# winddori2002/DEX-TTS

Hardware: AMD Instinct MI355X
Metric: mel-frames/s at n_timesteps=50, 80-ch mel (sampler only); RTF (higher is better)
Workload: dtype bf16; 1 GPU; gedex_b1: gedex_lj B=1/GPU T=512 n_timesteps=50 (BASELINE.json configs[1]); global_batch=1, frames=512, hipgraph=False, parallelism=1 GPU

## Files before the change

dex_tts_amd/csrc/conv3x3_bf16.hip:

```cpp
#include "kernels.h"
#include <cstdlib>
#include <cstdio>
#include "lp_util.h"
#include "kernels_lp.h"
#include "conv_gn.h"

namespace dex {
namespace DEX_LP_NS {

typedef float f32x16 __attribute__((ext_vector_type(16)));
typedef unsigned short u16;
typedef unsigned u32x4 __attribute__((ext_vector_type(4)));

__device__ __forceinline__ float cv_mish(float x) {
    const float e = __expf(fminf(x, 20.f));
    const float n = e * (e + 2.f);
    return x * (n * __builtin_amdgcn_rcpf(n + 2.f));
}

template <int NT, int COUT>
__device__ __forceinline__ void cv_epilogue(const Conv3P& p, f32x16 (&acc)[NT], int b, int ho, int w0, int nbase, int lane, int tid,
                                            long long* gnred) {
    const int i = lane & 31, hh = lane >> 5;
    constexpr int cpg = COUT / 8;
    if (p.gn_stats) { if (tid < 16) gnred[tid] = 0; __syncthreads(); }
    const bool full = ho < p.H && w0 + 32 <= p.W;
    const long ybase = (long)b * p.H * p.W * COUT + ((long)ho * p.W + w0 + 4 * hh) * COUT + nbase + i;
    float* yl = p.Y + ybase;
    u16* yh = reinterpret_cast<u16*>(p.Y) + ybase;
    const bool yb = p.y_bf16 != 0;
#pragma unroll
    for (int t = 0; t < NT; ++t) {
        const int n = nbase + t * 32 + i;
        const float bias = p.bias[n];
        float gs = 0.f, gss = 0.f;
        if (full && yb) {
            const bool odd = (lane & 1) != 0;
            u16* yp = yh + (odd ? 16 * COUT - 1 : 0) + t * 32;
#pragma unroll
            for (int r = 0; r < 16; ++r) { const float v = acc[t][r] + bias; gs += v; gss = fmaf(v, v, gss); }
#pragma unroll
            for (int j = 0; j < 8; ++j) {
                const float lo_r = acc[t][j] + bias, hi_r = acc[t][8 + j] + bias;
                const float recv = lane_xor1(odd ? lo_r : hi_r);
                const float mine = odd ? hi_r : lo_r;
                const unsigned pk = odd ? pack2_lp(recv, mine) : pack2_lp(mine, recv);
                *reinterpret_cast<unsigned*>(yp + ((j & 3) + 8 * (j >> 2)) * COUT) = pk;
            }
        } else if (full) {
            const bool odd = (lane & 1) != 0;
            float* yp = yl + (odd ? 16 * COUT - 1 : 0) + t * 32;
#pragma unroll
            for (int r = 0; r < 16; ++r) { const float v = acc[t][r] + bias; gs += v; gss = fmaf(v, v, gss); }
#pragma unroll
            for (int j = 0; j < 8; ++j) {
                const float lo_r = acc[t][j] + bias, hi_r = acc[t][8 + j] + bias;
                const float recv = lane_xor1(odd ? lo_r : hi_r);
                const float mine = odd ? hi_r : lo_r;
                *reinterpret_cast<float2*>(yp + ((j & 3) + 8 * (j >> 2)) * COUT) = odd ? make_float2(recv, mine) : make_float2(mine, recv);
            }
        } else {
#pragma unroll
            for (int r = 0; r < 16; ++r) {
                const int wo = w0 + (r & 3) + 8 * (r >> 2) + 4 * hh;
                const bool ok = ho < p.H && wo < p.W;
                const float v = acc[t][r] + bias;
                const float vs = ok ? v : 0.f;
                gs += vs; gss = fmaf(vs, vs, gss);
                if (ok) {
                    if (yb) yh[((r & 3) + 8 * (r >> 2)) * COUT + t * 32] = lp_bits(v);
                    else yl[((r & 3) + 8 * (r >> 2)) * COUT + t * 32] = v;
                }
            }
        }
        if (p.gn_stats) {
            for (int o = 1; o < cpg; o <<= 1) { gs += __shfl_xor(gs, o); gss += __shfl_xor(gss, o); }
            gs += __shfl_xor(gs, 32); gss += __shfl_xor(gss, 32);
            if (hh == 0 && (i & (cpg - 1)) == 0) {
                const double inv_n = 1.0 / ((double)p.H * p.W * cpg);
                gn_add(&gnred[(n / cpg) * 2], gn_fix(gs, inv_n)); gn_add(&gnred[(n / cpg) * 2 + 1], gn_fix(gss, inv_n));
            }
        }
    }
    if (p.gn_stats) {
        __syncthreads();
        if (tid < 16) {
            const long long v = gnred[tid];
            if (v != 0) {
                const int slot = (blockIdx.x + blockIdx.y * gridDim.x) % GN_SLOTS;
                gn_add(p.gn_stats + (((long)b * 8 + (tid >> 1)) * GN_SLOTS + slot) * 2 + (tid & 1), v);
            }
        }
    }
}

template <int NT, int COUT>
__device__ __forceinline__ void cv_res_store(const Conv3P& p, const f32x16 (&accr)[NT], int b, int ho, int w0, int nb, int lane) {
    const int i = lane & 31, hh = lane >> 5;
    float* yl = p.res_y + ((long)b * p.H * p.W + (long)ho * p.W + w0 + 4 * hh) * COUT + nb + i;
    const bool rfull = ho < p.H && w0 + 32 <= p.W;
    const bool odd = (lane & 1) != 0;
#pragma unroll
    for (int t = 0; t < NT; ++t) {
        const float bias = p.res_b[nb + t * 32 + i];
        if (rfull) {
            float* yp = yl + (odd ? 16 * COUT - 1 : 0) + t * 32;
#pragma unroll
            for (int j = 0; j < 8; ++j) {
                const float lo_r = accr[t][j] + bias, hi_r = accr[t][8 + j] + bias;
                const float recv = lane_xor1(odd ? lo_r : hi_r);
                const float mine = odd ? hi_r : lo_r;
                *reinterpret_cast<float2*>(yp + ((j & 3) + 8 * (j >> 2)) * COUT) = odd ? make_float2(recv, mine) : make_float2(mine, recv);
            }
        } else {
#pragma unroll
            for (int r = 0; r < 16; ++r) {
                const int wo = w0 + (r & 3) + 8 * (r >> 2) + 4 * hh;
                if (ho < p.H && wo < p.W) yl[((r & 3) + 8 * (r >> 2)) * COUT + t * 32] = accr[t][r] + bias;
            }
        }
    }
}

template <int CC, int COUT, int NSL, int TH, bool PRO2 = false, bool RES = false, bool XB = false, int NW = 4>
__global__ __launch_bounds__(64 * NW) void conv3x3_lp_kernel(const Conv3P p) {
    constexpr int PW = 34, PH = TH + 2;
    constexpr int LDP = CC + 8;
    constexpr int WN = NW / TH;
    constexpr int NTHR = 64 * NW;
    constexpr int NT = NSL / 32 / WN;
    constexpr int NSLICE = COUT / NSL;
    constexpr int ITEMS = PH * PW * (CC / 8);
    constexpr int NI = (ITEMS + NTHR - 1) / NTHR;
    constexpr int WPT = NSL * CC / 8 / NTHR;
    constexpr int RING = CC == 128 ? (PRO2 ? 1 : 2) : 3;
    constexpr int NPASS = CC == 128 ? (TH == 8 ? (PRO2 ? 8 : 4) : (PRO2 ? 5 : 2)) : (PRO2 ? 3 : 1);
    constexpr int NIP = (NI + NPASS - 1) / NPASS;
#ifdef DEX_LP_WSPLIT
    constexpr int NTAP = 18;
#else
    constexpr int NTAP = 9;
#endif
    static_assert(NT >= 1 && WPT >= 1, "tile");
    extern __shared__ __attribute__((aligned(16))) u16 smem[];
    u16* patch = smem;
    u16* wbuf = smem + PH * PW * LDP;
    u16* rbuf = wbuf + 2 * NSL * LDP;
    __shared__ long long gnred[16];
    constexpr int COEF_N = (TH == 8) ? 128 : 256;
    __shared__ __attribute__((aligned(16))) float coef[3][COEF_N];

    const int tid = threadIdx.x, lane = tid & 63, wave = tid >> 6;
    const int i = lane & 31, hh = lane >> 5;
    const int wrow = wave % TH, wcol = wave / TH;
#ifdef DEX_TIMING
    long long tk[8] = {0, 0, 0, 0, 0, 0, 0, 0};
    const long long tk0 = __builtin_readcyclecounter();
    long long tlast = tk0;
#define CSTAMP(k) do { const long long now_ = __builtin_readcyclecounter(); tk[k] += now_ - tlast; tlast = now_; } while (0)
#else
#define CSTAMP(k) do {} while (0)
#endif
    const int xs = p.skip_dead ? (int)((blockIdx.x + blockIdx.y + blockIdx.z) % gridDim.x) : (int)blockIdx.x;
    const int w0 = xs * 32, h0 = blockIdx.y * TH;
    const int b = blockIdx.z / NSLICE, slice = blockIdx.z % NSLICE;
    const int step = p.step;
    const float* X = p.X + (long)b * p.H * p.W * p.ldx + p.x_coff;
    const u16* Xh = reinterpret_cast<const u16*>(p.X) + (long)b * p.H * p.W * p.ldx + p.x_coff;
    const float* mrow = p.mask + (long)b * p.mask_bstride;
    const int K = 9 * p.Cin;
    const u16* Wg = reinterpret_cast<const u16*>(p.Wbf) + (long)slice * NSL * K;
    const bool pro = p.pro_stats != nullptr;
    if constexpr (!PRO2) {
        if (p.skip_dead) {
            const int wi = w0 - 1 + (lane < 34 ? lane : 33);
            const float mv = (unsigned)wi < (unsigned)p.W ? mrow[wi * p.mask_ws] : 0.f;
            if (__builtin_amdgcn_ballot_w64(mv != 0.f) == 0) {
                f32x16 zacc[NT];
#pragma unroll
                for (int t = 0; t < NT; ++t)
#pragma unroll
                    for (int r = 0; r < 16; ++r) zacc[t][r] = 0.f;
                if constexpr (RES) cv_res_store<NT, COUT>(p, zacc, b, h0 + wrow, w0, slice * NSL + wcol * NT * 32, lane);
                cv_epilogue<NT, COUT>(p, zacc, b, h0 + wrow, w0, slice * NSL + wcol * NT * 32, lane, tid, gnred);
                return;
            }
        }
    }

    f32x16 acc[NT];
#pragma unroll
    for (int t = 0; t < NT; ++t)
#pragma unroll
        for (int r = 0; r < 16; ++r) acc[t][r] = 0.f;

    f32x16 accr[RES ? NT : 1];
    if constexpr (RES) {
#pragma unroll
        for (int t = 0; t < NT; ++t)
#pragma unroll
            for (int r = 0; r < 16; ++r) accr[t][r] = 0.f;
    }
    int wofs[WPT], wlds[WPT];
#pragma unroll
    for (int j = 0; j < WPT; ++j) {
        const int it = tid + NTHR * j;
        const int n = it / (CC / 8), c8 = (it % (CC / 8)) * 8;
        wofs[j] = n * K + c8;
        wlds[j] = n * LDP + c8;
    }
    const int pc8 = (tid % (CC / 8)) * 8;

    CvGnLoads gnl{};
    if (pro) gnl = cv_gn_issue(p, b, tid, step);
    const int nchunk = p.Cin / CC;
    for (int ch = 0; ch < nchunk; ++ch) {
        const int cbase = ch * CC;
        u32x4 w0r[WPT], wr[RING][WPT], rwr[RES ? WPT : 1];
#ifdef DEX_LP_WSPLIT
        u32x4 rwl[RES ? WPT : 1];
#define WS_TAPOFS(t) ((long)((t) % 9) * p.Cin + ((t) >= 9 ? p.w_lo_off : 0L))
#else
#define WS_TAPOFS(t) ((long)(t) * p.Cin)
#endif
        float4 sc0, sc1, sh0, sh1, t0, t1;
#pragma unroll
        for (int ps = 0; ps < NPASS; ++ps) {
            float4 pf0[NIP], pf1[XB ? 1 : NIP], rf0[PRO2 ? NIP : 1], rf1[PRO2 ? NIP : 1];
            float pmk[NIP];
            bool pin[NIP];
#pragma unroll
            for (int q = 0; q < NIP; ++q) {
                const int it = min(tid + NTHR * (ps * NIP + q), ITEMS - 1);
                const int px = it / (CC / 8);
                const int pw = px % PW, ph = px / PW;
                const int hi = h0 + ph - 1, wi = w0 + pw - 1;
                const bool inb = (unsigned)hi < (unsigned)p.H && (unsigned)wi < (unsigned)p.W;
                const int hc = inb ? hi : 0, wc = inb ? wi : 0;
                if constexpr (XB) {
                    pf0[q] = *reinterpret_cast<const float4*>(Xh + ((long)hc * p.W + wc) * p.ldx + cbase + pc8);
                } else {
                    const float* src = X + ((long)hc * p.W + wc) * p.ldx + cbase + pc8;
                    pf0[q] = *reinterpret_cast<const float4*>(src);
                    pf1[q] = *reinterpret_cast<const float4*>(src + 4);
                }
                if constexpr (PRO2) {
                    const float* rs = p.pro_res + ((long)b * p.H * p.W + (long)hc * p.W + wc) * p.Cin + cbase + pc8;
                    rf0[q] = *reinterpret_cast<const float4*>(rs);
                    rf1[q] = *reinterpret_cast<const float4*>(rs + 4);
                }
                const float mk = mrow[wc * p.mask_ws];
                pmk[q] = inb ? mk : 0.f;
                pin[q] = inb;
            }
            if (ps == 0) {
                if constexpr (RES) {
                    const u16* Rg = reinterpret_cast<const u16*>(p.res_w) + (long)slice * NSL * p.Cin;
#pragma unroll
                    for (int j = 0; j < WPT; ++j) {
                        const int it = tid + NTHR * j;
                        rwr[j] = *reinterpret_cast<const u32x4*>(Rg + (long)(it / (CC / 8)) * p.Cin + cbase + (it % (CC / 8)) * 8);
#ifdef DEX_LP_WSPLIT
                        rwl[j] = *reinterpret_cast<const u32x4*>(Rg + p.res_lo_off + (long)(it / (CC / 8)) * p.Cin + cbase + (it % (CC / 8)) * 8);
#endif
                    }
                }
#pragma unroll
                for (int j = 0; j < WPT; ++j) w0r[j] = *reinterpret_cast<const u32x4*>(Wg + wofs[j] + cbase);
#pragma unroll
                for (int s = 0; s < RING; ++s)
#pragma unroll
                    for (int j = 0; j < WPT; ++j) wr[s][j] = *reinterpret_cast<const u32x4*>(Wg + wofs[j] + WS_TAPOFS(s + 1) + cbase);
                CSTAMP(0);
                if (pro && ch == 0) cv_gn_finish<COEF_N>(p, gnl, tid, coef);
                __builtin_amdgcn_sched_barrier(0);
                lds_barrier();
                CSTAMP(1);
                if (pro) {
                    const int c = cbase + pc8;
                    sc0 = *reinterpret_cast<const float4*>(&coef[0][c]); sc1 = *reinterpret_cast<const float4*>(&coef[0][c + 4]);
                    sh0 = *reinterpret_cast<const float4*>(&coef[1][c]); sh1 = *reinterpret_cast<const float4*>(&coef[1][c + 4]);
                    t0 = *reinterpret_cast<const float4*>(&coef[2][c]); t1 = *reinterpret_cast<const float4*>(&coef[2][c + 4]);
                }
            }
#pragma unroll
            for (int q = 0; q < NIP; ++q) {
                float4 f0, f1;
                if constexpr (XB) {
                    const float4 r = pf0[q];
                    const unsigned u0 = __float_as_uint(r.x), u1 = __float_as_uint(r.y), u2 = __float_as_uint(r.z), u3 = __float_as_uint(r.w);
                    f0 = make_float4(lp_lo(u0), lp_hi(u0), lp_lo(u1), lp_hi(u1));
                    f1 = make_float4(lp_lo(u2), lp_hi(u2), lp_lo(u3), lp_hi(u3));
                } else { f0 = pf0[q]; f1 = pf1[q]; }
#ifdef DEX_SCALAR_PROLOGUE
                if (pro) {
                    f0.x = cv_mish(fmaf(f0.x, sc0.x, sh0.x)) + t0.x; f0.y = cv_mish(fmaf(f0.y, sc0.y, sh0.y)) + t0.y;
                    f0.z = cv_mish(fmaf(f0.z, sc0.z, sh0.z)) + t0.z; f0.w = cv_mish(fmaf(f0.w, sc0.w, sh0.w)) + t0.w;
                    f1.x = cv_mish(fmaf(f1.x, sc1.x, sh1.x)) + t1.x; f1.y = cv_mish(fmaf(f1.y, sc1.y, sh1.y)) + t1.y;
                    f1.z = cv_mish(fmaf(f1.z, sc1.z, sh1.z)) + t1.z; f1.w = cv_mish(fmaf(f1.w, sc1.w, sh1.w)) + t1.w;
                }
#else
                if (pro) {
                    const f32x2 a0 = mish2_add(f32x2{f0.x, f0.y} * f32x2{sc0.x, sc0.y} + f32x2{sh0.x, sh0.y}, f32x2{t0.x, t0.y});
                    const f32x2 a1 = mish2_add(f32x2{f0.z, f0.w} * f32x2{sc0.z, sc0.w} + f32x2{sh0.z, sh0.w}, f32x2{t0.z, t0.w});
                    const f32x2 a2 = mish2_add(f32x2{f1.x, f1.y} * f32x2{sc1.x, sc1.y} + f32x2{sh1.x, sh1.y}, f32x2{t1.x, t1.y});
                    const f32x2 a3 = mish2_add(f32x2{f1.z, f1.w} * f32x2{sc1.z, sc1.w} + f32x2{sh1.z, sh1.w}, f32x2{t1.z, t1.w});
                    f0 = make_float4(a0.x, a0.y, a1.x, a1.y); f1 = make_float4(a2.x, a2.y, a3.x, a3.y);
                }
#endif
                const float mk = pmk[q];
                const int it = tid + NTHR * (ps * NIP + q);
                if constexpr (PRO2) {
                    f0.x = fmaf(f0.x, mk, rf0[q].x); f0.y = fmaf(f0.y, mk, rf0[q].y); f0.z = fmaf(f0.z, mk, rf0[q].z); f0.w = fmaf(f0.w, mk, rf0[q].w);
                    f1.x = fmaf(f1.x, mk, rf1[q].x); f1.y = fmaf(f1.y, mk, rf1[q].y); f1.z = fmaf(f1.z, mk, rf1[q].z); f1.w = fmaf(f1.w, mk, rf1[q].w);
                    const int px_ = it / (CC / 8), pw_ = px_ % PW, ph_ = px_ / PW;
                    if (slice == 0 && it < ITEMS && pin[q] && ph_ >= 1 && ph_ <= TH && pw_ >= 1 && pw_ <= 32) {
                        float* xo = p.pro_xout + ((long)b * p.H * p.W + (long)(h0 + ph_ - 1) * p.W + (w0 + pw_ - 1)) * p.Cin + cbase + pc8;
                        *reinterpret_cast<float4*>(xo) = f0;
                        *reinterpret_cast<float4*>(xo + 4) = f1;
                    }
                }
                uint4 v;
                v.x = pack2_lp(f0.x * mk, f0.y * mk); v.y = pack2_lp(f0.z * mk, f0.w * mk);
                v.z = pack2_lp(f1.x * mk, f1.y * mk); v.w = pack2_lp(f1.z * mk, f1.w * mk);
                if (it < ITEMS) *reinterpret_cast<uint4*>(patch + (it / (CC / 8)) * LDP + pc8) = v;
            }
        }
#pragma unroll
        for (int j = 0; j < WPT; ++j) *reinterpret_cast<u32x4*>(wbuf + wlds[j]) = w0r[j];
        if constexpr (RES) {
#pragma unroll
            for (int j = 0; j < WPT; ++j) *reinterpret_cast<u32x4*>(rbuf + wlds[j]) = rwr[j];
        }
        CSTAMP(2);
#pragma unroll
        for (int tt = 0; tt < NTAP; ++tt) {
            const int tap = tt % 9;
            lds_barrier();
            if (tt + 1 < NTAP) {
                u16* wn = wbuf + ((tt + 1) & 1) * NSL * LDP;
#pragma unroll
                for (int j = 0; j < WPT; ++j) *reinterpret_cast<u32x4*>(wn + wlds[j]) = wr[tt % RING][j];
                if (tt + 1 + RING < NTAP) {
#pragma unroll
                    for (int j = 0; j < WPT; ++j)
                        wr[tt % RING][j] = *reinterpret_cast<const u32x4*>(Wg + wofs[j] + WS_TAPOFS(tt + 1 + RING) + cbase);
                }
                __builtin_amdgcn_sched_barrier(0);
            }
#ifdef DEX_LP_WSPLIT
            if constexpr (RES) {
                if (tt == 5) {
#pragma unroll
                    for (int j = 0; j < WPT; ++j) *reinterpret_cast<u32x4*>(rbuf + wlds[j]) = rwl[j];
                }
            }
#endif
            const u16* wb = wbuf + (tt & 1) * NSL * LDP;
            const int kh = tap / 3, kw = tap - kh * 3;
            const u16* ap = patch + ((wrow + kh) * PW + i + kw) * LDP + hh * 8;
            const u16* bp = wb + (wcol * NT * 32 + i) * LDP + hh * 8;
#pragma unroll
            for (int ks = 0; ks < CC / 16; ++ks) {
                const lp8 af = *reinterpret_cast<const lp8*>(ap + ks * 16);
#pragma unroll
                for (int t = 0; t < NT; ++t) {
                    const lp8 bf = *reinterpret_cast<const lp8*>(bp + t * 32 * LDP + ks * 16);
                    acc[t] = DEX_MFMA_LP(af, bf, acc[t], 0, 0, 0);
                }
                if constexpr (RES) {
                    if (tap == 4) {
#pragma unroll
                        for (int t = 0; t < NT; ++t) {
                            const lp8 rf = *reinterpret_cast<const lp8*>(rbuf + (wcol * NT * 32 + t * 32 + i) * LDP + hh * 8 + ks * 16);
                            accr[t] = DEX_MFMA_LP(af, rf, accr[t], 0, 0, 0);
                        }
                    }
                }
            }
        }
    }
    if constexpr (RES) cv_res_store<NT, COUT>(p, accr, b, h0 + wrow, w0, slice * NSL + wcol * NT * 32, lane);
    CSTAMP(3);
    cv_epilogue<NT, COUT>(p, acc, b, h0 + wrow, w0, slice * NSL + wcol * NT * 32, lane, tid, gnred);
#ifdef DEX_TIMING
    CSTAMP(4);
    if (p.dbg && tid == 0) {
        long long* d = p.dbg + ((long)(blockIdx.z * gridDim.y + blockIdx.y) * gridDim.x + blockIdx.x) * 8;
        for (int k = 0; k < 5; ++k) d[k] = tk[k];
        d[7] = __builtin_readcyclecounter() - tk0;
    }
#endif
}

template <int CC, int COUT, int NSL, int TH, bool PRO2 = false, bool RES = false, bool XB = false, int NW = 4>
static void launch_c3(const Conv3P& p, hipStream_t st) {
    constexpr int LDP = CC + 8;
    const size_t lds = ((size_t)(TH + 2) * 34 * LDP + (2 + (RES ? 1 : 0)) * NSL * LDP) * sizeof(u16);
    static bool attr = false;
    if (!attr) {
        hipFuncSetAttribute(reinterpret_cast<const void*>(&conv3x3_lp_kernel<CC, COUT, NSL, TH, PRO2, RES, XB, NW>), hipFuncAttributeMaxDynamicSharedMemorySize, (int)lds);
        attr = true;
    }
    dim3 grid((p.W + 31) / 32, (p.H + TH - 1) / TH, p.B * (COUT / NSL));
    Conv3P q = p;
    q.skip_dead = (p.B >= 4 && (long)grid.x * grid.y * grid.z >= 1024 && knob_or("DEX_CONV_SKIP_DEAD", 1) != 0) ? 1 : 0;
    static char sym[96];
    if (!sym[0]) snprintf(sym, sizeof sym, "conv3x3_lp_kernel<%d,%d,%d,%d,%d,%d,%d,%d>", CC, COUT, NSL, TH, (int)PRO2, (int)RES, (int)XB, NW);
    g_last_symbol = sym;
    hipLaunchKernelGGL((conv3x3_lp_kernel<CC, COUT, NSL, TH, PRO2, RES, XB, NW>), grid, dim3(64 * NW), lds, st, q);
}

bool conv3x3_bf16_tail_supported(int C) {
#if defined(DEX_LP_WSPLIT) && !defined(DEX_WS_HAVE_CONV3)
    return false;
#endif
    return C == 64 || C == 128; }
bool conv3x3_bf16_xb_supported(int Cin, int Cout) {
#if defined(DEX_LP_WSPLIT) && !defined(DEX_WS_HAVE_CONV3)
    return false;
#endif
    return Cin == Cout && (Cin == 64 || Cin == 128); }
bool conv3x3_bf16_res_supported(int Cin, int Cout) {
#if defined(DEX_LP_WSPLIT) && !defined(DEX_WS_HAVE_CONV3_RES)
    return false;
#endif
    return (Cout == 128 && Cin == 64) || (Cout == 64 && (Cin == 128 || Cin == 256)); }
bool conv3x3_bf16_supported(int Cin, int Cout) {
#if defined(DEX_LP_WSPLIT) && !defined(DEX_WS_HAVE_CONV3)
    return false;
#endif
   
    return (Cin == 64 || Cin == 128 || Cin == 256) && (Cout == 64 || Cout == 128);
}

bool conv3x3_plain_lp_in_supported(int H, int W, int B, int Cin, int Cout) {
#if defined(DEX_LP_WSPLIT) && !defined(DEX_WS_HAVE_CONV3)
    return false;
#endif
   
    const int w8 = knob_or("DEX_CONV_W8", 1);
    const long tiles4 = (long)((W + 31) / 32) * ((H + 3) / 4) * B;
    return w8 && tiles4 >= 256 && Cin == 64 && Cout == 128;
}

bool conv3x3_cat_lp_in_supported(int H, int W, int B, int Cin, int Cout) {
#if defined(DEX_LP_WSPLIT) && !defined(DEX_WS_HAVE_CONV3_RES)
    return false;
#endif
   
    if (Cout != 64 || Cin < 128 || Cin % 128 != 0) return false;
    const int w8 = knob_or("DEX_CONV_W8", 1);
    const long small_max = knob_or("DEX_CONV_SMALL_MAX", 256);
    const long tiles4 = (long)((W + 31) / 32) * ((H + 3) / 4) * B;
    return w8 && tiles4 >= small_max;
}

void launch_conv3x3_lp(const Conv3P& p, hipStream_t st) {
    if (const int tpw = conv3x3_stream_tiles(p)) { launch_conv3x3_stream(p, tpw, st); return; }
    if (conv3x3_regw_form(p)) { launch_conv3x3_regw(p, st); return; }
    const bool tail_ = p.pro_res != nullptr;
    const long tiles4 = (long)((p.W + 31) / 32) * ((p.H + 3) / 4) * p.B;
    const long small_max = knob_or("DEX_CONV_SMALL_MAX", 256);
    const bool small = tiles4 < small_max;
    const int w8 = knob_or("DEX_CONV_W8", 1);
    const int th8 = knob_or("DEX_CONV_TH8", 1);
    if (th8 && w8 && !small && !tail_ && p.Cin == 128 && p.Cout == 128 && !p.res_w && p.H % 8 == 0 && (long)((p.W + 31) / 32) * (p.H / 8) * p.B >= 512) {
        p.x_bf16 ? launch_c3<128, 128, 128, 8, false, false, true, 8>(p, st) : launch_c3<128, 128, 128, 8, false, false, false, 8>(p, st);
        return;
    }
    if (w8 && !small && p.Cin == 128 && p.Cout == 128 && !p.res_w) {
        if (p.x_bf16) { tail_ ? launch_c3<128, 128, 128, 4, true, false, true, 8>(p, st) : launch_c3<128, 128, 128, 4, false, false, true, 8>(p, st); }
        else { tail_ ? launch_c3<128, 128, 128, 4, true, false, false, 8>(p, st) : launch_c3<128, 128, 128, 4, false, false, false, 8>(p, st); }
        return;
    }
    if (w8 && !small && p.res_w && p.Cout == 128 && p.Cin == 64) {
        p.x_bf16 ? launch_c3<64, 128, 128, 4, false, true, true, 8>(p, st) : launch_c3<64, 128, 128, 4, false, true, false, 8>(p, st);
        return;
    }
    if (th8 && w8 && !small && p.res_w && p.Cout == 64 && p.Cin >= 128 && !p.pro_stats && p.H % 8 == 0 && (long)((p.W + 31) / 32) * (p.H / 8) * p.B >= 512) {
        p.x_bf16 ? launch_c3<128, 64, 64, 8, false, true, true, 8>(p, st) : launch_c3<128, 64, 64, 8, false, true, false, 8>(p, st);
        return;
    }
    if (w8 && !small && p.res_w && p.Cout == 64 && p.Cin >= 128) {
        p.x_bf16 ? launch_c3<128, 64, 64, 4, false, true, true, 8>(p, st) : launch_c3<128, 64, 64, 4, false, true, false, 8>(p, st);
        return;
    }
    if (p.x_bf16) {
        if (tail_) {
            if (p.Cin == 64) { small ? launch_c3<64, 64, 64, 2, true, false, true>(p, st) : launch_c3<64, 64, 64, 4, true, false, true>(p, st); }
            else { small ? launch_c3<128, 128, 64, 2, true, false, true>(p, st) : launch_c3<128, 128, 128, 4, true, false, true>(p, st); }
        } else {
            if (p.Cin == 64) { small ? launch_c3<64, 64, 64, 2, false, false, true>(p, st) : launch_c3<64, 64, 64, 4, false, false, true>(p, st); }
            else { small ? launch_c3<128, 128, 64, 2, false, false, true>(p, st) : launch_c3<128, 128, 128, 4, false, false, true>(p, st); }
        }
        return;
    }
    if (tail_) {
        if (p.Cin == 64 && p.Cout == 64) { small ? launch_c3<64, 64, 64, 2, true>(p, st) : launch_c3<64, 64, 64, 4, true>(p, st); }
        else { small ? launch_c3<128, 128, 64, 2, true>(p, st) : launch_c3<128, 128, 128, 4, true>(p, st); }
        return;
    }
    if (p.res_w) {
        if (p.Cout == 128 && p.Cin == 64) { small ? launch_c3<64, 128, 64, 2, false, true>(p, st) : launch_c3<64, 128, 128, 4, false, true>(p, st); return; }
        if (p.Cout == 64 && p.Cin >= 128) { small ? launch_c3<128, 64, 64, 2, false, true>(p, st) : launch_c3<128, 64, 64, 4, false, true>(p, st); return; }
    }
    if (p.Cout == 64) {
        if (p.Cin == 64) { small ? launch_c3<64, 64, 64, 2>(p, st) : launch_c3<64, 64, 64, 4>(p, st); }
        else { small ? launch_c3<128, 64, 64, 2>(p, st) : launch_c3<128, 64, 64, 4>(p, st); }
    } else {
        if (p.Cin == 64) { small ? launch_c3<64, 128, 64, 2>(p, st) : launch_c3<64, 128, 128, 4>(p, st); }
        else { small ? launch_c3<128, 128, 64, 2>(p, st) : launch_c3<128, 128, 128, 4>(p, st); }
    }
}

}
}
```

dex_tts_amd/csrc/dex_api.hip:

```cpp
#include <hip/hip_runtime.h>
#include <cstdlib>

#include <cmath>
#include <cstdarg>
#include <atomic>
#include <cstdio>
#include <mutex>
#include <cstring>
#include <map>
#include <unordered_map>
#include <string_view>
#include <string>
#include <vector>

#include "../../include/dex_amd.h"
#include "kernels.h"
#include "weight_store.h"

using namespace dex;

namespace dex {
namespace {
const char* const KNOB_NAMES[] = {
    "DEX_CONV_STREAM", "DEX_CONV_PP", "DEX_CONV_SKIP_DEAD", "DEX_H_BF16", "DEX_ATTN_SEPARATE", "DEX_ATTN_Q64", "DEX_ATTN_Q64_TAIL", "DEX_ATTN_Q64_HALF", "DEX_DIT_XCDS", "DEX_ATTN_GENERIC", "DEX_RES2", "DEX_LP_INTER", "DEX_DIT_CHAIN",
    "DEX_DIT_CLUSTER", "DEX_DIT_CLUSTER_LOCAL", "DEX_ATTN_X_LP", "DEX_RES_X_LP", "DEX_CAT_LP", "DEX_XCD_MAP", "DEX_DEBUG_DROP_HANDOFF", "DEX_PATCH_FUSED",
    "DEX_CONV_DOWN", "DEX_CONVT_UP", "DEX_DEBUG_PLAN",
    "DEX_ATTN_SHARED_W8", "DEX_CONVT_MT", "DEX_CONVT_WGS", "DEX_CONV_DOWN_WGS", "DEX_CONV_REGW", "DEX_CONV_REGW_RES", "DEX_CONV_SMALL_MAX", "DEX_CONV_TH8",
    "DEX_CONV_W8", "DEX_DWCONV_CAP", "DEX_FINAL_CAP", "DEX_FIRST_CAP", "DEX_FIRST_MFMA", "DEX_GEMM_NWALK", "DEX_NWALK_SPLIT", "DEX_NWALK_BM", "DEX_POS_COL", "DEX_POS_COL_MIN",
    "DEX_POS_CT", "DEX_REGW_MIN_TILES", "DEX_REGW_WGS", "DEX_ROWCHAIN64", "DEX_ROWCHAIN64A", "DEX_TIV_CAP", "DEX_TV_CHAIN", "DEX_TIV_FOLD", "DEX_LINATTN_NSUB", "DEX_TV_FOLD", "DEX_OUT2_MIN", "DEX_NWALK_DMA",
    "DEX_LINATTN_HEADWAVES", "DEX_LINATTN_OUT2_HW"};
constexpr int N_KNOBS = (int)(sizeof(KNOB_NAMES) / sizeof(KNOB_NAMES[0]));
int knob_parse(const char* e) {
    if (!e) return KNOB_UNSET;
    char* end = nullptr;
    const long v = strtol(e, &end, 10);
    if (end == e) {
        static bool warned = false;
        if (!warned) { warned = true; fprintf(stderr, "libdexamd: ignoring a DEX_* knob whose value '%s' is not an integer\n", e); }
        return KNOB_UNSET;
    }
    return (int)v;
}
struct KnobSnapshot {
    int v[N_KNOBS];
    KnobSnapshot() { for (int i = 0; i < N_KNOBS; ++i) v[i] = knob_parse(getenv(KNOB_NAMES[i])); }
};
thread_local const KnobSnapshot* t_knobs = nullptr;
struct WsplitScope {
    bool prev;
    explicit WsplitScope(bool on) : prev(g_lp_wsplit) { g_lp_wsplit = on; }
    ~WsplitScope() { g_lp_wsplit = prev; }
};
struct KnobScope {
    const KnobSnapshot* prev;
    explicit KnobScope(const KnobSnapshot* k) : prev(t_knobs) { t_knobs = k; }
    ~KnobScope() { t_knobs = prev; }
};
}
static int knob_index(const char* name) {
    static const std::unordered_map<std::string_view, int> idx = [] {
        std::unordered_map<std::string_view, int> m;
        for (int i = 0; i < N_KNOBS; ++i) m.emplace(KNOB_NAMES[i], i);
        return m;
    }();
    const auto it = idx.find(std::string_view(name));
    return it == idx.end() ? -1 : it->second;
}
int knob(const char* name) {
    if (t_knobs) {
        const int i = knob_index(name);
        if (i >= 0) return t_knobs->v[i];
    }
    return knob_parse(getenv(name));
}
}
static_assert(PREC_FP32 == DEX_PREC_FP32 && PREC_BF16 == DEX_PREC_BF16 && PREC_FP16 == DEX_PREC_FP16 && PREC_FP16X2 == DEX_PREC_FP16X2, "kernels.h mirrors DexPrecision");

namespace {
void xcd_map_probe();

struct TD { float* p; int ld; int coff; int C; int lp = 0; };

struct ResW { const float *w1, *b1, *g1, *be1, *w2, *b2, *g2, *be2, *wr, *br, *mlp_w, *mlp_b; int cin, cout; };
constexpr int ATT_KSPLIT_MAX = 4;
static int att_split_cap(long tokens) { return tokens <= 20480 ? 8 : ATT_KSPLIT_MAX; }
static bool attention_q64_regime(int N, int B) {
    if (N < 1024) return dit_sep64_small_n(N, B) && dit_rowchain64_form(N, B, 0);
    const int ks = attention_q64_ksplit(N, B, att_split_cap((long)B * N));
    const int nt32 = (N + 31) / 32, ng = (nt32 + 7) / 8;
    return 2L * B * ng * ks >= 128;
}
struct LinW { const float *wqkv, *wqkv_raw, *wout_raw, *bias_eff, *g; const void *wq_lp[3], *wkv_lp[3], *wq_frag[3]; int C; };
struct DitBlockW { const float *wqkv, *bqkv, *wproj, *bproj, *wfc1, *bfc1, *wfc2, *bfc2, *ada_w, *ada_b; };

struct Prof { std::string name; hipEvent_t a, b; double flops, bytes; };
struct ProfAgg { std::string name; int calls; double ms, flops, bytes; };

struct Arena {
    char* base = nullptr; size_t off = 0, cap = 0; bool dry = true;
    void* take(size_t bytes) {
        off = (off + 255) & ~size_t(255);
        void* p = dry ? nullptr : (void*)(base + off);
        if (!dry && trace) fprintf(stderr, "plan[%d] off %zu bytes %zu\n", trace++, off, bytes);
        off += bytes;
        return p;
    }
    int trace = 0;
    float* f(size_t n) { return (float*)take(n * sizeof(float)); }
};

}

struct DexCtx : WeightStore {
    DexCtx() : WeightStore("") {}
    DexConfig cfg{};
    std::map<const float*, const void*> lp_of_[3];
    std::map<const float*, const void*> frag_of_[3];
    std::map<const void*, long> lo_off_;
    long lo_off(const void* twin) const { auto it = lo_off_.find(twin); return it == lo_off_.end() ? 0 : it->second; }
    int lpi() const { return precision == DEX_PREC_FP16X2 ? 2 : precision == DEX_PREC_FP16 ? 1 : 0; }
    int lp_kind() const { return precision == DEX_PREC_BF16 ? 1 : 2; }
    bool lp() const { return precision != DEX_PREC_FP32; }
    const std::map<const float*, const void*>& lp_of() const { return lp_of_[lpi()]; }
    const std::map<const float*, const void*>& frag_of() const { return frag_of_[lpi()]; }
    bool tuned = true;
    int precision = DEX_PREC_FP32;
    std::vector<std::vector<ResW>> down_res, up_res;
    std::vector<LinW> down_lin, up_lin;
    std::vector<const float*> down_ds_w, down_ds_b;
    std::vector<const float*> up_us_w, up_us_b;
    const float *fc_w3 = nullptr, *fc_w1 = nullptr;
    const float *fin_w = nullptr, *fin_b = nullptr, *fin_g = nullptr, *fin_be = nullptr, *fconv_w = nullptr, *fconv_b = nullptr;
    const float *pe_dw = nullptr, *pe_db = nullptr, *pe_pw = nullptr, *pe_pb = nullptr, *pos_w = nullptr, *pos_b = nullptr, *freq_pos = nullptr;
    const void* pos_wfrag[3] = {nullptr, nullptr, nullptr};
    std::vector<DitBlockW> blocks;
    const float *fl_w = nullptr, *fl_b = nullptr, *fl_ada_w = nullptr, *fl_ada_b = nullptr;
    const float *tv_wq_raw = nullptr, *tv_wk = nullptr, *tv_wv = nullptr, *tv_wl = nullptr;
    float *mel_basis = nullptr, *mel_filt = nullptr; void* mel_ws = nullptr; size_t mel_ws_bytes = 0;
    const int* last_xerr = nullptr;
    int* st_host = nullptr; hipEvent_t st_ev = nullptr; bool st_pending = false;
    struct Tap { std::string name; const float* p; std::vector<int64_t> shape; };
    std::vector<Tap> taps;
    bool prof_on = false;
    std::vector<Prof> prof;
    std::vector<ProfAgg> prof_agg;
    struct GraphEntry { std::vector<uint64_t> key; hipGraphExec_t exec; uint64_t stamp; const int* xerr; };
    std::vector<GraphEntry> graphs;
    uint64_t graph_clock = 0;
    void drop_graphs() { for (auto& g : graphs) hipGraphExecDestroy(g.exec); graphs.clear(); }
};

namespace {

int stage_dim(const DexConfig& c, int i) { return c.dim * c.dim_mults[i]; }
int in_planes(const DexConfig& c) { return 2 + (c.n_spks > 1 ? 1 : 0); }
int mid_dim(const DexConfig& c) { return stage_dim(c, c.n_stages - 1); }
int mid_h(const DexConfig& c) { return c.n_feats >> (c.n_stages - 1); }
int grid_h(const DexConfig& c) { return mid_h(c) / c.dit_stride; }
int token_rows(const DexConfig& c) { return (mid_h(c) + 2 * (c.dit_patch / 2) - c.dit_patch) / c.dit_stride + 1; }
int token_cols(const DexConfig& c, int wmid) {
    const int p = c.dit_patch, s = c.dit_stride;
    const int wp = (wmid % p == 0) ? wmid : wmid + (p - wmid % p);
    return (wp + 2 * (p / 2) - p) / s + 1;
}
int mlp_hidden(const DexConfig& c) { return (int)(c.dit_hidden * c.dit_mlp_ratio); }

void add_resnet(DexCtx* x, const std::string& p, int cin, int cout, int tdim) {
    x->add(p + ".mlp.1.weight", {cout, tdim}); x->add(p + ".mlp.1.bias", {cout});
    for (int blk = 1; blk <= 2; ++blk) {
        const std::string q = p + ".block" + std::to_string(blk) + ".block";
        x->add(q + ".0.weight", {cout, blk == 1 ? cin : cout, 3, 3}); x->add(q + ".0.bias", {cout});
        x->add(q + ".1.weight", {cout}); x->add(q + ".1.bias", {cout});
    }
    if (cin != cout) { x->add(p + ".res_conv.weight", {cout, cin, 1, 1}); x->add(p + ".res_conv.bias", {cout}); }
}
void add_linattn(DexCtx* x, const std::string& p, int c) {
    x->add(p + ".fn.g", {1});
    x->add(p + ".fn.fn.to_qkv.weight", {384, c, 1, 1});
    x->add(p + ".fn.fn.to_out.weight", {c, 128, 1, 1});
    x->add(p + ".fn.fn.to_out.bias", {c});
}
void build_inventory(DexCtx* x) {
    const DexConfig& c = x->cfg;
    const int d = c.dim;
    x->add("mlp.0.weight", {4 * d, d}); x->add("mlp.0.bias", {4 * d});
    x->add("mlp.2.weight", {d, 4 * d}); x->add("mlp.2.bias", {d});
    if (c.variant == DEX_VARIANT_DEX)
        for (const char* n : {"mlp_adap", "mlp_adap_sty"}) {
            const std::string s(n);
            x->add(s + ".0.weight", {d, d}); x->add(s + ".0.bias", {d});
            x->add(s + ".2.weight", {2 * d, d}); x->add(s + ".2.bias", {2 * d});
        }
    if (c.n_spks > 1) {
        const int e = c.spk_emb_dim;
        x->add("spk_mlp.0.weight", {4 * e, e}); x->add("spk_mlp.0.bias", {4 * e});
        x->add("spk_mlp.2.weight", {c.n_feats, 4 * e}); x->add("spk_mlp.2.bias", {c.n_feats});
    }
    for (int i = 0; i < c.n_stages; ++i) {
        const int ci = i == 0 ? in_planes(c) : stage_dim(c, i - 1), co = stage_dim(c, i);
        const std::string p = "downs." + std::to_string(i);
        add_resnet(x, p + ".0", ci, co, d); add_resnet(x, p + ".1", co, co, d); add_linattn(x, p + ".2", co);
        if (i < c.n_stages - 1) { x->add(p + ".3.conv.weight", {co, co, 3, 3}); x->add(p + ".3.conv.bias", {co}); }
    }
    const int hid = c.dit_hidden, mid = mid_dim(c), mh = mlp_hidden(c);
    x->add("vit.freq_new_pos_embed", {1, hid, grid_h(c), 1});
    x->add("vit.x_embedder.proj.0.weight", {mid, 1, c.dit_patch, c.dit_patch}); x->add("vit.x_embedder.proj.0.bias", {mid});
    x->add("vit.x_embedder.proj.2.weight", {hid, mid, 1, 1}); x->add("vit.x_embedder.proj.2.bias", {hid});
    x->add("vit.t_embedder.mlp.0.weight", {hid, 256}); x->add("vit.t_embedder.mlp.0.bias", {hid});
    x->add("vit.t_embedder.mlp.2.weight", {hid, hid}); x->add("vit.t_embedder.mlp.2.bias", {hid});
    x->add("vit.pos_conv.0.weight", {hid, hid / c.dit_conv_pos_groups, c.dit_conv_pos, c.dit_conv_pos});
    x->add("vit.pos_conv.0.bias", {hid});
    for (int k = 0; k < c.dit_depth; ++k) {
        const std::string p = "vit.blocks." + std::to_string(k);
        x->add(p + ".attn.qkv.weight", {3 * hid, hid}); x->add(p + ".attn.qkv.bias", {3 * hid});
        x->add(p + ".attn.proj.weight", {hid, hid}); x->add(p + ".attn.proj.bias", {hid});
        x->add(p + ".mlp.fc1.weight", {mh, hid}); x->add(p + ".mlp.fc1.bias", {mh});
        x->add(p + ".mlp.fc2.weight", {hid, mh}); x->add(p + ".mlp.fc2.bias", {hid});
        x->add(p + ".adaLN_modulation.1.weight", {6 * hid, hid}); x->add(p + ".adaLN_modulation.1.bias", {6 * hid});
    }
    const int so = c.dit_stride * c.dit_stride * mid;
    x->add("vit.final_layer.linear.weight", {so, hid}); x->add("vit.final_layer.linear.bias", {so});
    x->add("vit.final_layer.adaLN_modulation.1.weight", {2 * hid, hid}); x->add("vit.final_layer.adaLN_modulation.1.bias", {2 * hid});
    if (c.variant == DEX_VARIANT_DEX) {
        for (const char* w : {"w_q", "w_k", "w_v", "linear"}) x->add(std::string("tv_adaptor.") + w + ".weight", {mid, mid});
        for (const char* s : {"mean_sap", "std_sap"}) {
            x->add(std::string("tiv_adaptor.") + s + ".W.weight", {1, mid});
            x->add(std::string("tiv_adaptor.") + s + ".W.bias", {1});
        }
    }
    for (int j = 0; j < c.n_stages - 1; ++j) {
        const int i = c.n_stages - 1 - j;
        const int ci = stage_dim(c, i - 1), co = stage_dim(c, i);
        const std::string p = "ups." + std::to_string(j);
        add_resnet(x, p + ".0", co * 2, ci, d); add_resnet(x, p + ".1", ci, ci, d); add_linattn(x, p + ".2", ci);
        x->add(p + ".3.conv.weight", {ci, ci, 4, 4}); x->add(p + ".3.conv.bias", {ci});
    }
    x->add("final_block.block.0.weight", {d, d, 3, 3}); x->add("final_block.block.0.bias", {d});
    x->add("final_block.block.1.weight", {d}); x->add("final_block.block.1.bias", {d});
    x->add("final_conv.weight", {1, d, 1, 1}); x->add("final_conv.bias", {1});
}

__global__ void pack_convt_kernel(const float* src, float* dst, int Cin, int Cout) {
    const long total = 4L * 4 * Cin * Cout;
    for (long i = (long)blockIdx.x * blockDim.x + threadIdx.x; i < total; i += (long)gridDim.x * blockDim.x) {
        const int co = (int)(i % Cout);
        const int ci = (int)((i / Cout) % Cin);
        const int tap = (int)((i / ((long)Cout * Cin)) % 4);
        const int par = (int)(i / ((long)Cout * Cin * 4));
        const int ph = par >> 1, pw = par & 1, th = tap >> 1, tw = tap & 1;
        const int kh = (ph ? 0 : 1) + 2 * th, kw = (pw ? 0 : 1) + 2 * tw;
        dst[i] = src[(((long)ci * Cout + co) * 4 + kh) * 4 + kw];
    }
}

}

extern "C" {

const char* dex_version(void) { return "dexamd 0.1 (gfx950)"; }

int dex_ctx_create(const DexConfig* cfg, DexCtx** out) {
    if (!cfg || !out) return DEX_ERR_ARG;
    DexCtx* x = new DexCtx();
    x->cfg = *cfg;
    const DexConfig& c = x->cfg;
    *out = x;
    if (c.n_feats != 80) return x->fail(DEX_ERR_ARG, "n_feats must be 80 (diffusion.py:226 hard-codes it)");
    if (c.n_stages < 2 || c.n_stages > 4) return x->fail(DEX_ERR_ARG, "n_stages must be in [2,4]");
    if (c.dim != 64 && c.dim != 128) return x->fail(DEX_ERR_ARG, "dim must be 64 (GeDEX, DEX-VCTK/ESD) or 128 (DEX-LibriTTS)");
    if (c.dit_heads < 1 || c.dit_hidden % c.dit_heads || !attention_head_dim_supported(c.dit_hidden / c.dit_heads))
        return x->fail(DEX_ERR_ARG, "DiT head_dim must be 64, 128, 192 or 256 (hidden %d heads %d)", c.dit_hidden, c.dit_heads);
    if (c.dit_hidden % 64 || c.dit_hidden > 512) return x->fail(DEX_ERR_ARG, "dit_hidden must be a multiple of 64, <= 512");
    if (mlp_hidden(c) % 64) return x->fail(DEX_ERR_ARG, "mlp hidden must be a multiple of 64");
    if (c.dit_conv_pos_groups < 1 || c.dit_hidden % c.dit_conv_pos_groups || (c.dit_hidden / c.dit_conv_pos_groups) % 16 ||
        c.dit_hidden / c.dit_conv_pos_groups > 64)
        return x->fail(DEX_ERR_ARG, "pos-conv groups must be 16, 32, 48 or 64 channels wide");
    if (c.dit_conv_pos % 2) return x->fail(DEX_ERR_ARG, "conv_pos must be even");
    if (c.variant == DEX_VARIANT_DEX && !attention_head_dim_supported(mid_dim(c)))
        return x->fail(DEX_ERR_ARG, "DEX adaptors need mid_dim 64, 128, 192 or 256 (the cross-attention's head_dim)");
    x->tuned = c.dim == 64 && c.dit_hidden == 256 && c.dit_heads == 2 && c.dit_hidden / c.dit_conv_pos_groups == 32 &&
               (c.variant != DEX_VARIANT_DEX || mid_dim(c) == 128);
    build_inventory(x);
    xcd_map_probe();
    return DEX_OK;
}

void dex_ctx_destroy(DexCtx* x) {
    if (!x) return;
    x->release();
    if (x->mel_basis) hipFree(x->mel_basis);
    if (x->mel_filt) hipFree(x->mel_filt);
    if (x->mel_ws) hipFree(x->mel_ws);
    x->drop_graphs();
    for (auto& pr : x->prof) { hipEventDestroy(pr.a); hipEventDestroy(pr.b); }
    if (x->st_ev) hipEventDestroy(x->st_ev);
    if (x->st_host) hipHostFree(x->st_host);
    delete x;
}

const char* dex_last_error(const DexCtx* x) { return x ? x->err.c_str() : "null context"; }
int dex_ctx_num_weights(const DexCtx* x) { return x ? (int)x->keys.size() : 0; }

int dex_ctx_weight_info(const DexCtx* x, int i, const char** key, int64_t shape[4], int* ndim) { return x ? x->info(i, key, shape, ndim) : DEX_ERR_ARG; }
int dex_ctx_load_weight(DexCtx* x, const char* key, const float* w_dev, const int64_t* shape, int ndim) {
    return x ? x->load(key, w_dev, shape, ndim, nullptr, true) : DEX_ERR_ARG;
}
int dex_ctx_load_weight_async(DexCtx* x, const char* key, const float* w_dev, const int64_t* shape, int ndim, dex_stream_t stream) {
    return x ? x->load(key, w_dev, shape, ndim, (hipStream_t)stream, false) : DEX_ERR_ARG;
}

int dex_ctx_set_precision(DexCtx* x, int precision) {
    if (!x || (precision != DEX_PREC_FP32 && precision != DEX_PREC_BF16 && precision != DEX_PREC_FP16 && precision != DEX_PREC_FP16X2)) return DEX_ERR_ARG;
    x->precision = precision;
    return DEX_OK;
}

}

void dex::slaney_mel_filterbank(float* filt) {
    const int nb = 513;
    const int n_mels = 80; const double sr = 22050, fmin = 0, fmax = 8000;
    auto hz2mel = [](double f) { const double fsp = 200.0 / 3; return f >= 1000.0 ? 1000.0 / fsp + log(f / 1000.0) / (log(6.4) / 27.0) : f / fsp; };
    auto mel2hz = [](double m) { const double fsp = 200.0 / 3, mlm = 1000.0 / fsp; return m >= mlm ? 1000.0 * exp(log(6.4) / 27.0 * (m - mlm)) : fsp * m; };
    std::vector<double> mf(n_mels + 2);
    const double m0 = hz2mel(fmin), m1 = hz2mel(fmax);
    for (int i = 0; i < n_mels + 2; ++i) mf[i] = mel2hz(m0 + (m1 - m0) * i / (n_mels + 1));
    for (int i = 0; i < n_mels; ++i) {
        const double enorm = 2.0 / (mf[i + 2] - mf[i]);
        for (int k = 0; k < nb; ++k) {
            const double fr = (sr / 2.0) * k / (nb - 1);
            const double lower = (fr - mf[i]) / (mf[i + 1] - mf[i]), upper = (mf[i + 2] - fr) / (mf[i + 2] - mf[i + 1]);
            const double w = fmax > 0 ? std::max(0.0, std::min(lower, upper)) : 0.0;
            filt[(size_t)i * nb + k] = (float)(w * enorm);
// ... 1535 lines not shown
```

Baseline: 27610 mel-frames/s.

## Add 5-row conv3x3 tile variants so the grid fits in a single CU wave

Adds a TH=5 row tile configuration for the 64-channel and 64->128 residual conv3x3 kernels, using 10 or 5 waves per block. A launch heuristic picks it when the current tiling needs more than one round of blocks across the CUs but the 5-row tiling fits within one round while filling at least three quarters of them. This removes the tail of a second partial wave of blocks. Weight staging now handles weight item counts that do not divide evenly by thread count, using per-item guards, at the cost of some predication overhead. Timing-only debug code also records the hardware ID and XCC ID.

```diff
diff --git a/dex_tts_amd/csrc/conv3x3_bf16.hip b/dex_tts_amd/csrc/conv3x3_bf16.hip
--- a/dex_tts_amd/csrc/conv3x3_bf16.hip
+++ b/dex_tts_amd/csrc/conv3x3_bf16.hip
@@ -132,16 +132,19 @@
     constexpr int NSLICE = COUT / NSL;
     constexpr int ITEMS = PH * PW * (CC / 8);
     constexpr int NI = (ITEMS + NTHR - 1) / NTHR;
-    constexpr int WPT = NSL * CC / 8 / NTHR;
+    constexpr int WITEMS = NSL * CC / 8;
+    constexpr int WPT = (WITEMS + NTHR - 1) / NTHR;
+    constexpr bool WFULL = WITEMS % NTHR == 0;
     constexpr int RING = CC == 128 ? (PRO2 ? 1 : 2) : 3;
-    constexpr int NPASS = CC == 128 ? (TH == 8 ? (PRO2 ? 8 : 4) : (PRO2 ? 5 : 2)) : (PRO2 ? 3 : 1);
+    constexpr int NPASS = TH == 5 ? (CC == 128 ? (PRO2 ? 6 : 3) : (PRO2 ? 3 : XB ? 1 : 2))
+                                  : CC == 128 ? (TH == 8 ? (PRO2 ? 8 : 4) : (PRO2 ? 5 : 2)) : (PRO2 ? 3 : 1);
     constexpr int NIP = (NI + NPASS - 1) / NPASS;
 #ifdef DEX_LP_WSPLIT
     constexpr int NTAP = 18;
 #else
     constexpr int NTAP = 9;
 #endif
-    static_assert(NT >= 1 && WPT >= 1, "tile");
+    static_assert(NT >= 1 && WPT >= 1 && NW % TH == 0 && NTHR % (CC / 8) == 0, "tile");
     extern __shared__ __attribute__((aligned(16))) u16 smem[];
     u16* patch = smem;
     u16* wbuf = smem + PH * PW * LDP;
@@ -202,12 +205,14 @@
             for (int r = 0; r < 16; ++r) accr[t][r] = 0.f;
     }
     int wofs[WPT], wlds[WPT];
+    bool wok[WPT];
 #pragma unroll
     for (int j = 0; j < WPT; ++j) {
         const int it = tid + NTHR * j;
         const int n = it / (CC / 8), c8 = (it % (CC / 8)) * 8;
         wofs[j] = n * K + c8;
         wlds[j] = n * LDP + c8;
+        wok[j] = WFULL || it < WITEMS;
     }
     const int pc8 = (tid % (CC / 8)) * 8;
 
@@ -259,6 +264,7 @@
 #pragma unroll
                     for (int j = 0; j < WPT; ++j) {
                         const int it = tid + NTHR * j;
+                        if (!wok[j]) continue;
                         rwr[j] = *reinterpret_cast<const u32x4*>(Rg + (long)(it / (CC / 8)) * p.Cin + cbase + (it % (CC / 8)) * 8);
 #ifdef DEX_LP_WSPLIT
                         rwl[j] = *reinterpret_cast<const u32x4*>(Rg + p.res_lo_off + (long)(it / (CC / 8)) * p.Cin + cbase + (it % (CC / 8)) * 8);
@@ -266,11 +272,11 @@
                     }
                 }
 #pragma unroll
-                for (int j = 0; j < WPT; ++j) w0r[j] = *reinterpret_cast<const u32x4*>(Wg + wofs[j] + cbase);
+                for (int j = 0; j < WPT; ++j) if (wok[j]) w0r[j] = *reinterpret_cast<const u32x4*>(Wg + wofs[j] + cbase);
 #pragma unroll
                 for (int s = 0; s < RING; ++s)
 #pragma unroll
-                    for (int j = 0; j < WPT; ++j) wr[s][j] = *reinterpret_cast<const u32x4*>(Wg + wofs[j] + WS_TAPOFS(s + 1) + cbase);
+                    for (int j = 0; j < WPT; ++j) if (wok[j]) wr[s][j] = *reinterpret_cast<const u32x4*>(Wg + wofs[j] + WS_TAPOFS(s + 1) + cbase);
                 CSTAMP(0);
                 if (pro && ch == 0) cv_gn_finish<COEF_N>(p, gnl, tid, coef);
                 __builtin_amdgcn_sched_barrier(0);
@@ -327,10 +333,10 @@
             }
         }
 #pragma unroll
-        for (int j = 0; j < WPT; ++j) *reinterpret_cast<u32x4*>(wbuf + wlds[j]) = w0r[j];
+        for (int j = 0; j < WPT; ++j) if (wok[j]) *reinterpret_cast<u32x4*>(wbuf + wlds[j]) = w0r[j];
         if constexpr (RES) {
 #pragma unroll
-            for (int j = 0; j < WPT; ++j) *reinterpret_cast<u32x4*>(rbuf + wlds[j]) = rwr[j];
+            for (int j = 0; j < WPT; ++j) if (wok[j]) *reinterpret_cast<u32x4*>(rbuf + wlds[j]) = rwr[j];
         }
         CSTAMP(2);
 #pragma unroll
@@ -340,11 +346,11 @@
             if (tt + 1 < NTAP) {
                 u16* wn = wbuf + ((tt + 1) & 1) * NSL * LDP;
 #pragma unroll
-                for (int j = 0; j < WPT; ++j) *reinterpret_cast<u32x4*>(wn + wlds[j]) = wr[tt % RING][j];
+                for (int j = 0; j < WPT; ++j) if (wok[j]) *reinterpret_cast<u32x4*>(wn + wlds[j]) = wr[tt % RING][j];
                 if (tt + 1 + RING < NTAP) {
 #pragma unroll
                     for (int j = 0; j < WPT; ++j)
-                        wr[tt % RING][j] = *reinterpret_cast<const u32x4*>(Wg + wofs[j] + WS_TAPOFS(tt + 1 + RING) + cbase);
+                        if (wok[j]) wr[tt % RING][j] = *reinterpret_cast<const u32x4*>(Wg + wofs[j] + WS_TAPOFS(tt + 1 + RING) + cbase);
                 }
                 __builtin_amdgcn_sched_barrier(0);
             }
@@ -352,7 +358,7 @@
             if constexpr (RES) {
                 if (tt == 5) {
 #pragma unroll
-                    for (int j = 0; j < WPT; ++j) *reinterpret_cast<u32x4*>(rbuf + wlds[j]) = rwl[j];
+                    for (int j = 0; j < WPT; ++j) if (wok[j]) *reinterpret_cast<u32x4*>(rbuf + wlds[j]) = rwl[j];
                 }
             }
 #endif
@@ -388,6 +394,10 @@
     if (p.dbg && tid == 0) {
         long long* d = p.dbg + ((long)(blockIdx.z * gridDim.y + blockIdx.y) * gridDim.x + blockIdx.x) * 8;
         for (int k = 0; k < 5; ++k) d[k] = tk[k];
+        unsigned hw, xcc;
+        asm volatile("s_getreg_b32 %0, hwreg(HW_REG_HW_ID)" : "=s"(hw));
+        asm volatile("s_getreg_b32 %0, hwreg(HW_REG_XCC_ID)" : "=s"(xcc));
+        d[5] = hw; d[6] = xcc & 15u;
         d[7] = __builtin_readcyclecounter() - tk0;
     }
 #endif
@@ -454,6 +464,32 @@
     const long small_max = knob_or("DEX_CONV_SMALL_MAX", 256);
     const long tiles4 = (long)((W + 31) / 32) * ((H + 3) / 4) * B;
     return w8 && tiles4 >= small_max;
+}
+
+static bool launch_c3_round1(const Conv3P& p, bool small, hipStream_t st) {
+    if (!knob_or("DEX_CONV_ROUND1", 1)) return false;
+    const bool tail_ = p.pro_res != nullptr;
+#ifdef DEX_LP_WSPLIT
+    const bool c64 = p.Cin == 64 && p.Cout == 64 && !p.res_w && !tail_;
+#else
+    const bool c64 = p.Cin == 64 && p.Cout == 64 && !p.res_w;
+#endif
+    const bool r128 = p.Cin == 64 && p.Cout == 128 && p.res_w && !tail_ && !p.x_bf16;
+    if (!c64 && !r128) return false;
+    const long strips = (long)((p.W + 31) / 32) * p.B;
+    const long cur = c64 ? strips * (small ? (p.H + 1) / 2 : (p.H + 3) / 4) : strips * (small ? (p.H + 1) / 2 * 2 : (p.H + 3) / 4);
+    const long one = strips * ((p.H + 4) / 5) * (c64 ? 1 : 4);
+    const long ncu = device_cus();
+    if (cur <= ncu || one > ncu || one * 4 < ncu * 3) return false;
+    if (c64) {
+#ifndef DEX_LP_WSPLIT
+        if (tail_) { p.x_bf16 ? launch_c3<64, 64, 64, 5, true, false, true, 10>(p, st) : launch_c3<64, 64, 64, 5, true, false, false, 10>(p, st); return true; }
+#endif
+        p.x_bf16 ? launch_c3<64, 64, 64, 5, false, false, true, 10>(p, st) : launch_c3<64, 64, 64, 5, false, false, false, 10>(p, st);
+    } else {
+        launch_c3<64, 128, 32, 5, false, true, false, 5>(p, st);
+    }
+    return true;
 }
 
 void launch_conv3x3_lp(const Conv3P& p, hipStream_t st) {
@@ -486,6 +522,7 @@
         p.x_bf16 ? launch_c3<128, 64, 64, 4, false, true, true, 8>(p, st) : launch_c3<128, 64, 64, 4, false, true, false, 8>(p, st);
         return;
     }
+    if (launch_c3_round1(p, small, st)) return;
     if (p.x_bf16) {
         if (tail_) {
             if (p.Cin == 64) { small ? launch_c3<64, 64, 64, 2, true, false, true>(p, st) : launch_c3<64, 64, 64, 4, true, false, true>(p, st); }
diff --git a/dex_tts_amd/csrc/dex_api.hip b/dex_tts_amd/csrc/dex_api.hip
--- a/dex_tts_amd/csrc/dex_api.hip
+++ b/dex_tts_amd/csrc/dex_api.hip
@@ -28,7 +28,7 @@
     "DEX_ATTN_SHARED_W8", "DEX_CONVT_MT", "DEX_CONVT_WGS", "DEX_CONV_DOWN_WGS", "DEX_CONV_REGW", "DEX_CONV_REGW_RES", "DEX_CONV_SMALL_MAX", "DEX_CONV_TH8",
     "DEX_CONV_W8", "DEX_DWCONV_CAP", "DEX_FINAL_CAP", "DEX_FIRST_CAP", "DEX_FIRST_MFMA", "DEX_GEMM_NWALK", "DEX_NWALK_SPLIT", "DEX_NWALK_BM", "DEX_POS_COL", "DEX_POS_COL_MIN",
     "DEX_POS_CT", "DEX_REGW_MIN_TILES", "DEX_REGW_WGS", "DEX_ROWCHAIN64", "DEX_ROWCHAIN64A", "DEX_TIV_CAP", "DEX_TV_CHAIN", "DEX_TIV_FOLD", "DEX_LINATTN_NSUB", "DEX_TV_FOLD", "DEX_OUT2_MIN", "DEX_NWALK_DMA",
-    "DEX_LINATTN_HEADWAVES", "DEX_LINATTN_OUT2_HW"};
+    "DEX_LINATTN_HEADWAVES", "DEX_LINATTN_OUT2_HW", "DEX_CONV_ROUND1"};
 constexpr int N_KNOBS = (int)(sizeof(KNOB_NAMES) / sizeof(KNOB_NAMES[0]));
 int knob_parse(const char* e) {
     if (!e) return KNOB_UNSET;
```

After: 28470 mel-frames/s, median of 6. 3.1% higher.
